# kepengxu/RealCamNet

Hardware: AMD Instinct MI355X
Metric: megapixels/sec RAW->sRGB at 4K (higher is better)
Workload: dtype bf16; 1 GPU; cfg3: 3840x2160 Bayer mosaic -> unshuffle+pad16 -> LiteISPNet_GFM_LSC_GMA -> sRGB 3840x2160, 8 frames/GPU, bf16 storage / fp32 accumulate; frames_per_gpu=8, global_frames=8, parallelism=frame-shard x1, collective=none

## Files before the change

### realcamnet_amd/csrc/conv.hip

```cpp
#include <mutex>
#include <vector>

#include "conv32_kernel.hpp"

namespace rc {

struct ConvPlan {
    int ck = 0, nt = 0, unit = 0, upt = 0, nu = 0, steps = 0;
    int n_chunks = 0, n_ct = 0, cout_packed = 0;
    int m32 = 0;
};

static int g_persist_on = 1;
extern int g_dw3_seg16;
extern int g_dec_lds;
extern int g_wmsa_mfma;
extern int g_pw_grid_cap;
static int g_pss = 0;
static int g_poison = 0;
static int g_thin = 2;
static int g_auto = 1;
static int g_sums_compact = 1;
static int g_conv32 = 0;

static bool make_plan(int cin, int cout, int ksize, int dtype, int out_mode, ConvPlan* p, int cout_tile = 0) {
    if (cin < 1 || cout < 1 || (ksize != 1 && ksize != 3 && ksize != 2 && ksize != 5)) return false;
    if (dtype != RC_F32 && dtype != RC_BF16 && dtype != RC_F16) return false;
    const bool h16 = dtype != RC_F32;
    if (ksize == 5 && (cout > 16 || out_mode == RC_OUT_PIXEL_SHUFFLE2 || (h16 ? (cin % 48 != 0 && cin % 32 != 0) : cin % 16 != 0))) return false;
    if (out_mode == RC_OUT_PIXEL_SHUFFLE2_NCHW && cout % 4 != 0) return false;
    if (ksize == 2 && (dtype != RC_BF16 || cin % 16 != 0 || out_mode != RC_OUT_NHWC || (cin % 48 == 0 && cin % 64 != 0))) return false;
    p->unit = dtype == RC_F32 ? 4 : 8;
    if (ksize == 5) p->ck = h16 ? (cin % 48 == 0 ? 48 : 32) : 16;
    else if (h16) {
        if (cin <= 8) p->ck = 8;
        else if (ksize == 1 && cin % 80 == 0 && cin % 64 != 0) p->ck = 80;
        else if (ksize >= 2 && cin % 64 == 0 && cin > 64) p->ck = 32;
        else if (cin % 64 == 0) p->ck = 64;
        else if (cin % 48 == 0) p->ck = 48;
        else if (ksize == 3 && cin == 32) p->ck = 32;
        else if (ksize == 3 && cin % 32 == 0 && cin > 64) p->ck = 32;
        else p->ck = 16;
    } else {
        p->ck = cin <= 4 ? 4 : 16;
    }
    if (out_mode == RC_OUT_PIXEL_SHUFFLE2) {
        if (cout % 4 != 0) return false;
        const int cps = cout / 4;
        if (cps % 64 == 0 && !(cps % 48 == 0 && h16 && cin == 48)) p->nt = 4;
        else if (cps % 48 == 0) p->nt = 3;
        else if (cps % 64 == 0) p->nt = 4;
        else if (cps % 16 == 0) p->nt = 1;
        else return false;
// ... 181 lines not shown
                    for (int dx = 0; dx < 3; ++dx) {
                        const int a = i + dy - 1, b = j + dx - 1;
                        const int fy = a < 0 ? -1 : a >> 1, ii = a & 1, fx = b < 0 ? -1 : b >> 1, jj = b & 1;
                        for (int cc = 0; cc < c; ++cc) {
                            const int m = 4 * cc + 2 * ii + jj;
                            const double v2 = w2[(((size_t)oo * c + cc) * 3 + dy) * 3 + dx];
                            if (b1) bacc[row] += v2 * (double)b1[m];
                            for (int k = 0; k < c; ++k)
                                for (int ey = 0; ey < 3; ++ey)
                                    for (int ex = 0; ex < 3; ++ex)
                                        acc[(((size_t)row * c + k) * 5 + (fy + ey + 1)) * 5 + (fx + ex + 1)] += v2 * (double)w1[(((size_t)m * c + k) * 3 + ey) * 3 + ex];
                        }
                    }
            }
    for (size_t n = 0; n < acc.size(); ++n) wc[n] = (float)acc[n];
    for (size_t n = 0; n < bacc.size(); ++n) bc[n] = (float)bacc[n];
    return RC_OK;
}

int rc_conv_sum_tiles(int height, int width) { return 4 * ceil_div(height, kTH) * ceil_div(width, kTW); }

int rc_debug_set(const char* key, int value) {
    RC_REQUIRE(key != nullptr, "rc_debug_set: null key");
    if (std::string(key) == "persist") { g_persist_on = value < 0 ? 0 : (value > 3 ? 3 : value); return RC_OK; }
    if (std::string(key) == "conv_flags") { g_dbg_flags = value; return RC_OK; }
    if (std::string(key) == "pair_impl") { g_pair_impl = value < 0 || value > 2 ? 0 : value; return RC_OK; }
    if (std::string(key) == "dec_lds") { g_dec_lds = value != 0; return RC_OK; }
    if (std::string(key) == "dw3_seg16") { g_dw3_seg16 = value != 0; return RC_OK; }
    if (std::string(key) == "wmsa_mfma") { g_wmsa_mfma = value != 0; return RC_OK; }
    if (std::string(key) == "pss") { g_pss = value != 0; return RC_OK; }
    if (std::string(key) == "sums_compact") { g_sums_compact = value != 0; return RC_OK; }
    if (std::string(key) == "persist_auto") { g_auto = value < 0 ? 0 : (value > 2 ? 2 : value); return RC_OK; }
    if (std::string(key) == "thin") { g_thin = value < 0 ? 0 : (value > 2 ? 2 : value); return RC_OK; }
    if (std::string(key) == "lds_poison") { g_poison = value != 0; return RC_OK; }
    if (std::string(key) == "conv32") { g_conv32 = value < 0 ? 0 : (value > 4 ? 4 : value); return RC_OK; }
    if (std::string(key) == "wino_nnt") { wino_set_nnt(value); return RC_OK; }
    if (std::string(key) == "pw_grid_cap") { g_pw_grid_cap = value <= 0 || value > (1 << 22) ? (1 << 22) : value; return RC_OK; }
    return fail(RC_ERR_INVALID, std::string("rc_debug_set: unknown key ") + key);
}

int rc_debug_get(const char* key) {
    if (key == nullptr) return -1;
    if (std::string(key) == "persist") return g_persist_on;
    if (std::string(key) == "conv32") return g_conv32;
    if (std::string(key) == "conv_flags") return g_dbg_flags;
    if (std::string(key) == "pss") return g_pss;
    if (std::string(key) == "sums_compact") return g_sums_compact;
    if (std::string(key) == "persist_auto") return g_auto;
    if (std::string(key) == "thin") return g_thin;
    if (std::string(key) == "lds_poison") return g_poison;
    if (std::string(key) == "wino_nnt") return wino_get_nnt();
    if (std::string(key) == "pw_grid_cap") return g_pw_grid_cap;
    return -1;
}

int rc_debug_set_ptr(const char* key, void* p) {
    RC_REQUIRE(key != nullptr, "rc_debug_set_ptr: null key");
    if (std::string(key) == "conv_phase_timing") { g_dbg_ptr = static_cast<long long*>(p); return RC_OK; }
    return fail(RC_ERR_INVALID, std::string("rc_debug_set_ptr: unknown key ") + key);
}

int rc_prof_enable(int on) {
    std::lock_guard<std::mutex> lk(g_prof_mu);
    for (auto& r : g_prof) { (void)hipEventDestroy(r.e0); (void)hipEventDestroy(r.e1); }
    g_prof.clear();
    g_prof_on = on != 0;
    return RC_OK;
}

int rc_prof_collect(int64_t* n_launches, double* total_ms, double* total_flops) {
    std::lock_guard<std::mutex> lk(g_prof_mu);
    double ms = 0.0, fl = 0.0;
    for (auto& r : g_prof) {
        RC_HIP_CHECK(hipEventSynchronize(r.e1));
        float t = 0.f;
        RC_HIP_CHECK(hipEventElapsedTime(&t, r.e0, r.e1));
        ms += t; fl += r.flops;
    }
    if (n_launches) *n_launches = (int64_t)g_prof.size();
    if (total_ms) *total_ms = ms;
    if (total_flops) *total_flops = fl;
    return RC_OK;
// ... 98 lines not shown
    a.cin_vec_ok = (d->cin % p.unit == 0) && aligned16(d->in0) && aligned16(d->in1) && aligned16(d->in_store) &&
                   (d->in_gate == nullptr || reinterpret_cast<uintptr_t>(d->in_gate) % 4 == 0);
    a.cin_chunk_ok = d->cin % p.ck == 0;
    a.fold2 = fold ? 1 : 0; a.src_H = d->src_h; a.src_W = d->src_w; a.cfold = d->cin / 4;
    a.in0 = d->in0; a.in1 = d->in1; a.in_gate = d->in_gate; a.in_store = d->in_store;
    a.wpacked = d->wpacked; a.bias = d->bias;
    a.film_scale = d->film_scale; a.film_shift = d->film_shift;
    a.act = d->act; a.act_slope = d->act_slope;
    a.mul_plus1 = d->mul_plus1; a.residual = d->residual; a.out_scale = d->out_scale;
    a.out = d->out; a.out_mode = d->out_mode; a.out_dtype = d->out_dtype; a.out_h = d->out_h; a.out_w = d->out_w;
    a.chan_sums = d->chan_sums; a.cout_packed = p.cout_packed;
    a.sum_slots = d->chan_sums_slots > 0 ? d->chan_sums_slots : 4 * ceil_div(d->height, kTH) * ceil_div(d->width, kTW);
    a.sums_compact = 0; a.query = nullptr; a.sums_compact_ok = g_sums_compact;
    {
        int key = (d->act == RC_ACT_RELU ? 1 : 0) | (d->act == RC_ACT_LEAKY ? 2 : 0) | (d->film_scale ? 4 : 0) |
                  (d->mul_plus1 ? 8 : 0) | (d->residual ? 16 : 0) | (d->chan_sums ? 32 : 0) | (d->out_scale ? 64 : 0);
        bool fast = full_tiles && d->out_mode != RC_OUT_NCHW && d->out_mode != RC_OUT_PIXEL_SHUFFLE2_NCHW && d->act != RC_ACT_GELU && d->act != RC_ACT_RELU_POST;
        if (d->act == RC_ACT_LEAKY) fast = fast && d->act_slope >= 0.f && d->act_slope <= 1.f;
        if (d->film_scale)
            fast = fast && d->cout % 4 == 0 && reinterpret_cast<uintptr_t>(d->film_scale) % 16 == 0 && reinterpret_cast<uintptr_t>(d->film_shift) % 16 == 0;
        if (d->out_scale) fast = fast && d->cout % 4 == 0 && reinterpret_cast<uintptr_t>(d->out_scale) % 16 == 0;
        switch (key) { case 0: case 1: case 2: case 16: case 32: case 8: case 6: case 33: case 34: case 80: break; default: fast = false; }
        a.ep_key = fast ? key : -1;
        a.pss = g_pss && d->out_mode == RC_OUT_PIXEL_SHUFFLE2 && !p.m32 && p.n_chunks == 1 && p.n_ct == 4 && d->cout == 4 * 16 * p.nt &&
                d->dtype == RC_BF16 && d->in_gate == nullptr && fast && (key == 0 || key == 1 || key == 2);
    }
    {
        const int num_cus = device_cu_count();
        a.num_cus = num_cus;
        a.persist_ok = g_persist_on;
        a.auto_impl = g_auto;
        a.thin = g_thin;
        a.dbg = g_dbg_ptr;
        a.dbg_flags = g_dbg_flags;
        a.td = make_tile_decode(a.tiles_x, a.tiles_y, kBandRows);
        a.td_wsm = make_tile_decode(a.tiles_x, (a.H + kWsmTH - 1) / kWsmTH, kBandRows);
        a.div_n_ct = make_magic(a.n_ct);
    }
    es_out = es;
    return RC_OK;
}

int rc_conv2d(const rc_conv_desc* d, void* stream_) {
    RC_REQUIRE(d != nullptr, "rc_conv2d: null desc");
    RC_REQUIRE(d->algo == 0 || d->algo == 1, "rc_conv2d: algo must be 0 (implicit GEMM) or 1 (Winograd F(2x2,3x3))");
    if (d->algo == 1) {
        if (g_poison) { if (int e = rc_debug_poison_lds(0x7FC07FC0u, stream_)) return e; }
        return wino_conv(d, as_stream(stream_));
    }
    ConvPlan p;
    ConvArgs a;
    size_t es = 0;
    if (int e = conv_build_args(d, p, a, es)) return e;
    hipStream_t stream = as_stream(stream_);
    if (g_poison) { if (int e = rc_debug_poison_lds(0x7FC07FC0u, stream_)) return e; }
    void* tok = nullptr;
    const double taps = d->ksize == 2 ? 9.0 / 4.0 : (double)d->ksize * d->ksize;
    const double px = (double)d->batch * d->height * d->width;
    const double osz = (d->out_mode == RC_OUT_NCHW || d->out_mode == RC_OUT_PIXEL_SHUFFLE2_NCHW) ? (d->out_dtype == RC_F32 ? 4.0 : 2.0) : (double)es;
    const double bytes = px * d->cin * es * (1.0 + (d->in1 ? 1.0 : 0.0) + (d->in_store ? 1.0 : 0.0)) + px * d->cout * osz +
                         px * d->cout * es * ((d->residual ? 1.0 : 0.0) + (d->mul_plus1 ? 1.0 : 0.0));
    conv_prof_begin(2.0 * px * (double)d->cin * d->cout * taps, stream, &tok, bytes, d->cin, d->cout, d->ksize);
    const int rcode = p.m32 ? (p.ck == 16 ? conv32_ck16(0, a, stream) : p.ck == 32 ? conv32_ck32(g_conv32 == 3 ? 1 : 0, a, stream) : conv32_ck48(0, a, stream))
                            : dispatch_conv(d->dtype, d->ksize, p.ck, p.nt, a, stream);
    conv_prof_end(tok, stream);
    return rcode;
}
// ... 17 lines not shown
```

### realcamnet_amd/csrc/conv_kernel.hpp

```cpp
#pragma once
#include "common.hpp"

namespace rc {

struct MagicDiv { unsigned m, sh; };
inline MagicDiv make_magic(int d) {
    if (d <= 1) return MagicDiv{0u, 0u};
    int L = 0;
    while ((2 << L) <= d) ++L;
    const unsigned long long m = ((1ull << (31 + L)) + (unsigned long long)d - 1) / (unsigned long long)d;
    return MagicDiv{(unsigned)m, (unsigned)(L - 1)};
}
__device__ __forceinline__ int magic_div(int n, const MagicDiv& d) {
    return d.m ? (int)(__umulhi((unsigned)n, d.m) >> d.sh) : n;
}
struct TileDecode { MagicDiv sp_total, band, last_rows; };
inline TileDecode make_tile_decode(int tiles_x, int tiles_y, int band_rows) {
    return TileDecode{make_magic(tiles_x * tiles_y), make_magic(band_rows * tiles_x), make_magic(tiles_y % band_rows ? tiles_y % band_rows : 1)};
}

struct ConvArgs {
    int batch, H, W, cin, cout;
    int n_chunks, n_ct, tiles_x, tiles_y;
    int cin_vec_ok;
    int cin_chunk_ok;
    const void* in0; const void* in1; const float* in_gate; void* in_store;
    const void* wpacked; const float* bias;
    const float* film_scale; const float* film_shift;
    int act; float act_slope;
    const void* mul_plus1; const void* residual;
    const float* out_scale;
    void* out; int out_mode; int out_dtype; int out_h, out_w;
    float* chan_sums; int cout_packed;
    int sum_slots;
    int sums_compact_ok;
    int sums_compact;
    int* query;
    int num_cus; int persist_ok;
    int ep_key;
    TileDecode td, td_wsm;
    MagicDiv div_n_ct;
    int w_resident;
    int pss;
    int auto_impl;
    int thin;
    int fold2, src_H, src_W, cfold;
    long long* dbg;
    int dbg_flags;
};

constexpr int kTH = 8, kTW = 32, kThreads = 256;

constexpr int pix_stride_bytes(int ck_bytes) {
    int s = (ck_bytes + 15) / 16 * 16;
    while (s % 64 != 32) s += 16;
    return s;
}

__host__ __device__ constexpr int unit_map_steps(int upt, int taps) {
    return upt == 6 ? taps + (taps + 1) / 2 : (taps * upt + 3) / 4;
}
__host__ __device__ constexpr bool unit_map(int upt, int taps, int s, int q, int& tap, int& cu) {
    if (upt == 6) {
        if (s < taps) { tap = s; cu = q; return true; }
        tap = 2 * (s - taps) + (q >> 1); cu = 4 + (q & 1);
        return tap < taps;
    }
    const int u = 4 * s + q;
    tap = u / upt; cu = u % upt;
    return u < taps * upt;
}

template <typename T, int CK_, int NT_, int KS_, int TH_ = kTH>
struct ConvCfg {
    using elem = T;
    static constexpr int CK = CK_, NT = NT_, KS = KS_, TH = TH_;
    static constexpr int UNIT = 16 / (int)sizeof(T);
    static_assert(CK % UNIT == 0, "CK must be a whole number of 16-byte units");
    static constexpr int UPT = CK / UNIT;
    static constexpr int TAPS = KS * KS;
    static constexpr int STEPS = unit_map_steps(UPT, TAPS);
    static constexpr int HALO = KS / 2;
// ... 80 lines not shown
            __builtin_amdgcn_raw_buffer_store_b64(u32x2_t{w[4 * NQ], w[4 * NQ + 1]}, r, voff + 16 * NQ, 0, 0);
    }
}

template <typename TT, int NV>
__device__ __forceinline__ void buf_load_row(__amdgpu_buffer_rsrc_t r, int voff, float* v) {
    if constexpr (sizeof(TT) == 4) {
#pragma unroll
        for (int i = 0; i < NV; i += 4) {
            const u32x4_t t = __builtin_amdgcn_raw_buffer_load_b128(r, voff + 4 * i, 0, 0);
            v[i] = __uint_as_float(t.x); v[i + 1] = __uint_as_float(t.y); v[i + 2] = __uint_as_float(t.z); v[i + 3] = __uint_as_float(t.w);
        }
    } else {
#pragma unroll
        for (int i = 0; i < NV; i += 4) {
            const u32x2_t p = __builtin_amdgcn_raw_buffer_load_b64(r, voff + 2 * i, 0, 0);
            v[i] = lo16<TT>(p.x); v[i + 1] = hi16<TT>(p.x);
            v[i + 2] = lo16<TT>(p.y); v[i + 3] = hi16<TT>(p.y);
        }
    }
}

constexpr int kBandRows = 8;
__device__ __forceinline__ void band_decode(int idx, int tiles_x, int tiles_y, const TileDecode& td, int& ty, int& tx) {
    const int band = magic_div(idx, td.band);
    const int rem = idx - band * (kBandRows * tiles_x);
    const int rows_left = tiles_y - band * kBandRows;
    const bool whole = rows_left >= kBandRows;
    const int col = whole ? rem >> 3 : magic_div(rem, td.last_rows);
    ty = band * kBandRows + (rem - col * (whole ? kBandRows : rows_left));
    tx = col;
}

template <class Cfg>
struct ConvDev {
    using T = typename Cfg::elem;
    using TS = typename std::conditional<sizeof(T) == 4, bf16_t, T>::type;
    static constexpr int CK = Cfg::CK, NT = Cfg::NT, KS = Cfg::KS, UNIT = Cfg::UNIT, UPT = Cfg::UPT, TAPS = Cfg::TAPS;
    static constexpr int STEPS = Cfg::STEPS, HALO = Cfg::HALO, THH = Cfg::THH, TWH = Cfg::TWH;
    static constexpr int SPIX = Cfg::SPIX, NV = 4 * NT, ES = (int)sizeof(T);
    static constexpr int VPP = UPT;
    static constexpr int NPIX = THH * TWH;
    static constexpr int PPP = kThreads / VPP;
    static constexpr int ACTIVE = PPP * VPP;
    static constexpr int NI = (NPIX + PPP - 1) / PPP;
    static constexpr bool TABLE = (UPT % 4 != 0) && (UPT != 6);

    __device__ static constexpr int tap_off(int tap) { return ((tap / KS) * TWH + (tap % KS)) * SPIX; }

    struct LaneOff {
        int a;
        int b;
        int c;
        int tab[TABLE ? STEPS : 1];
    };
    __device__ static __forceinline__ void lane_offsets(int q, LaneOff& lo) {
        lo.a = q * 16;
        lo.b = (q >> 1) * SPIX + (4 + (q & 1)) * 16;
        lo.c = (q >> 1) * (TWH - (KS - 1)) * SPIX + (4 + (q & 1)) * 16;
        if constexpr (TABLE) {
#pragma unroll
            for (int s = 0; s < STEPS; ++s) {
                int tap = 0, cu = 0;
                if (!unit_map(UPT, TAPS, s, q, tap, cu)) { tap = TAPS - 1; cu = UPT - 1; }
                lo.tab[s] = tap_off(tap) + cu * 16;
            }
        } else {
            lo.tab[0] = 0;
        }
    }
    __device__ static __forceinline__ int step_off(int s, const LaneOff& lo) {
        if constexpr (TABLE) {
            return lo.tab[s];
        } else if constexpr (UPT == 6) {
            if (s < TAPS) return lo.a + tap_off(s);
            const int t0 = 2 * (s - TAPS);
            const bool wrap = (t0 + 1 < TAPS) && ((t0 + 1) % KS == 0);
            return (wrap ? lo.c : lo.b) + tap_off(t0);
        } else {
            const int u = 4 * s;
            return lo.a + tap_off(u / UPT) + (u % UPT) * 16;
        }
    }
    __device__ static constexpr bool step_has_pad(int s) {
        int tap = 0, cu = 0;
        return !unit_map(UPT, TAPS, s, 3, tap, cu);
    }
    __device__ static __forceinline__ bool lane_is_pad(int s, int q) {
        if constexpr (UPT == 6) return q >= 2;
        else return 4 * s + q >= TAPS * UPT;
    }

    struct TileSrc {
        __amdgpu_buffer_rsrc_t r0, r1, rst;
        int gy0, gx0;
        int soff;
        bool interior;
// ... 73 lines not shown
        }
    }
    template <bool GATED>
    __device__ static __forceinline__ void load_tile_interior(const ConvArgs& a, const TileSrc& t, const TileOffs& to, int chunk,
                                                              uint4 (&r0)[NI], uint4 (&r1)[GATED ? NI : 1]) {
        const int soff = t.soff + chunk_soff(a, chunk);
#pragma unroll
        for (int k = 0; k < NI; ++k) {
            r0[k] = buf_load16(t.r0, to.o[k], soff);
            if constexpr (GATED) r1[k] = buf_load16(t.r1, to.o[k], soff);
        }
    }
    template <bool GATED>
    __device__ static __forceinline__ void load_tile_border(const ConvArgs& a, const TileSrc& t, int chunk, int tid,
                                                            uint4 (&r0)[NI], uint4 (&r1)[GATED ? NI : 1]) {
        const int v = tid % VPP, p0 = tid / VPP;
        const bool live = tid < ACTIVE;
#pragma unroll
        for (int k = 0; k < NI; ++k) {
            bool center;
            const int off = vec_off(a, t, chunk, p0 + k * PPP, v, live, center);
            r0[k] = buf_load16(t.r0, off, 0);
            if constexpr (GATED) r1[k] = buf_load16(t.r1, off, 0);
        }
    }

    template <bool GATED>
    __device__ static __forceinline__ void commit_tile(const ConvArgs& a, const TileSrc& t, const TileOffs& to, int chunk, int tid,
                                                       const uint4 (&r0)[NI], const uint4 (&r1)[GATED ? NI : 1],
                                                       const float (&gv)[GATED ? UNIT : 1], char* s_in) {
        const int v = tid % VPP, p0 = tid / VPP;
        const bool live = tid < ACTIVE;
        char* dst = s_in + p0 * SPIX + v * 16;
#pragma unroll
        for (int k = 0; k < NI; ++k) {
            const int pix = p0 + k * PPP;
            uint4 raw = r0[k];
            if constexpr (GATED) {
                float f0[UNIT], f1[UNIT];
                Vec16<T>::unpack(r0[k], f0);
                Vec16<T>::unpack(r1[k], f1);
#pragma unroll
                for (int e = 0; e < UNIT; ++e) f0[e] = f0[e] * gv[e] + f1[e];
                raw = Vec16<T>::pack(f0);
                if (t.interior) {
                    buf_store16(t.rst, to.ctr[k], t.soff + chunk * CK * ES, raw);
                } else {
                    bool center;
                    const int off = vec_off(a, t, chunk, pix, v, live, center);
                    buf_store16(t.rst, center ? off : kOOB, 0, raw);
                }
            }
            if (live && pix < NPIX) *reinterpret_cast<uint4*>(dst + k * PPP * SPIX) = raw;
        }
    }

    __device__ static __forceinline__ void stage_tile_scalar(const ConvArgs& a, int b, int y0, int x0, int chunk, int tid,
                                                             char* s_in, T* in_store) {
        const T* in0 = static_cast<const T*>(a.in0);
        const T* in1 = static_cast<const T*>(a.in1);
        const size_t img_base = (size_t)b * a.H * a.W;
        if constexpr (ES == 2 && UNIT == 8 && VPP == 1) {
            if (a.cin == 4 && a.in_gate == nullptr && (reinterpret_cast<uintptr_t>(in0) & 7) == 0) {
                for (int i = tid; i < NPIX; i += kThreads) {
                    const int py = i / TWH, px = i - py * TWH;
                    const int gy = y0 + py - HALO, gx = x0 + px - HALO;
// ... 21 lines not shown
                    if (c0 + e < a.cin) {
                        val = to_f32(in0[off + e]);
                        if (a.in_gate != nullptr)
                            val = val * a.in_gate[(size_t)b * a.cin + c0 + e] + to_f32(in1[off + e]);
                    }
                    f0[e] = val;
                }
                raw = Vec16<T>::pack(f0);
                if (a.in_gate != nullptr && in_store != nullptr && center) {
#pragma unroll
                    for (int e = 0; e < UNIT; ++e)
                        if (c0 + e < a.cin) in_store[off + e] = from_f32<T>(f0[e]);
                }
            }
            *reinterpret_cast<uint4*>(s_in + pix * SPIX + v * 16) = raw;
        }
    }

    __device__ static __forceinline__ void dma_weights(const char* src, char* dst, int nkb, int wave, int lane_w) {
        for (int kb = wave; kb < nkb; kb += kThreads / 64)
            __builtin_amdgcn_global_load_lds((const __attribute__((address_space(1))) void*)(src + kb * 1024 + lane_w),
                                             (__attribute__((address_space(3))) void*)(dst + kb * 1024), 16, 0, 0);
    }

    static constexpr int FR = NT + 4;
    static constexpr int FM = 4 * NT;
    template <int I>
    __device__ static __forceinline__ void load_frag_item(int s, int w0, const char* s_in, const char* s_w, int lane_x,
                                                          int lane_w, const LaneOff& lo, uint4 (&wf)[NT], uint4 (&xf)[4]) {
        if constexpr (I < NT) {
            wf[I] = *reinterpret_cast<const uint4*>(s_w + ((s - w0) * NT + I) * 1024 + lane_w);
        } else {
            constexpr int pt = I - NT;
            xf[pt] = *reinterpret_cast<const uint4*>(s_in + lane_x + step_off(s, lo) + ((pt >> 1) * TWH + (pt & 1) * 16) * SPIX);
        }
    }
    __device__ static __forceinline__ void zero_pad_frags(int s, int q, uint4 (&xf)[4]) {
        if (step_has_pad(s)) {
            if (lane_is_pad(s, q)) {
#pragma unroll
                for (int pt = 0; pt < 4; ++pt) xf[pt] = make_uint4(0u, 0u, 0u, 0u);
            }
        }
    }
    __device__ static __forceinline__ void load_frags(int s, int w0, const char* s_in, const char* s_w, int lane_x,
                                                      int lane_w, int q, const LaneOff& lo, uint4 (&wf)[NT], uint4 (&xf)[4]) {
#pragma unroll
        for (int nt = 0; nt < NT; ++nt)
            wf[nt] = *reinterpret_cast<const uint4*>(s_w + ((s - w0) * NT + nt) * 1024 + lane_w);
        const char* xp = s_in + lane_x + step_off(s, lo);
#pragma unroll
        for (int pt = 0; pt < 4; ++pt)
            xf[pt] = *reinterpret_cast<const uint4*>(xp + ((pt >> 1) * TWH + (pt & 1) * 16) * SPIX);
        zero_pad_frags(s, q, xf);
    }
    __device__ static __forceinline__ void mma_frags(const uint4 (&wf)[NT], const uint4 (&xf)[4], f32x4 (&acc)[4][NT]) {
#pragma unroll
        for (int pt = 0; pt < 4; ++pt)
#pragma unroll
            for (int nt = 0; nt < NT; ++nt) Mma<T>::run(wf[nt], xf[pt], acc[pt][nt]);
    }
    static constexpr int SLOTS = FM * (ES == 4 ? 4 : 1);
    __device__ static __forceinline__ void mma_slot(int m, const uint4 (&wf)[NT], const uint4 (&xf)[4], f32x4 (&acc)[4][NT]) {
        if constexpr (ES == 4) {
            const int e = m / FM, j = m % FM, pt = j / NT, nt = j % NT;
            const unsigned w = e == 0 ? wf[nt].x : e == 1 ? wf[nt].y : e == 2 ? wf[nt].z : wf[nt].w;
            const unsigned x = e == 0 ? xf[pt].x : e == 1 ? xf[pt].y : e == 2 ? xf[pt].z : xf[pt].w;
            acc[pt][nt] = __builtin_amdgcn_mfma_f32_16x16x4f32(__uint_as_float(w), __uint_as_float(x), acc[pt][nt], 0, 0, 0);
        } else {
            Mma<T>::run(wf[m % NT], xf[m / NT], acc[m / NT][m % NT]);
        }
    }
    template <int I, bool NEXT>
    __device__ static __forceinline__ void step_interleaved(int s, int w0, const char* s_in, const char* s_w, int lane_x, int lane_w,
                                                            const LaneOff& lo, const uint4 (&wf)[NT], const uint4 (&xf)[4],
                                                            uint4 (&wfn)[NT], uint4 (&xfn)[4], f32x4 (&acc)[4][NT]) {
        if constexpr (I < FR) {
            if constexpr (NEXT) load_frag_item<I>(s + 1, w0, s_in, s_w, lane_x, lane_w, lo, wfn, xfn);
            if constexpr (ES == 2) __builtin_amdgcn_sched_barrier(0);
#pragma unroll
            for (int m = (I * SLOTS) / FR; m < ((I + 1) * SLOTS) / FR; ++m) mma_slot(m, wf, xf, acc);
            if constexpr (ES == 2) __builtin_amdgcn_sched_barrier(0);
            step_interleaved<I + 1, NEXT>(s, w0, s_in, s_w, lane_x, lane_w, lo, wf, xf, wfn, xfn, acc);
        }
    }
    template <int S0, int COUNT, int W0, bool DBUF = true>
    __device__ static __forceinline__ void mma_steps(const char* s_in, const char* s_w, int lane_x, int lane_w, int q,
                                                     const LaneOff& lo, f32x4 (&acc)[4][NT]) {
        constexpr int END = (S0 + COUNT) < STEPS ? (S0 + COUNT) : STEPS;
        if constexpr (S0 < END && !DBUF) {
#pragma unroll
            for (int s = S0; s < END; ++s) {
                uint4 wf[NT], xf[4];
                load_frags(s, W0, s_in, s_w, lane_x, lane_w, q, lo, wf, xf);
                mma_frags(wf, xf, acc);
            }
        } else if constexpr (S0 < END && ES == 4) {
            uint4 wfa[NT], xfa[4], wfb[NT], xfb[4];
            load_frags(S0, W0, s_in, s_w, lane_x, lane_w, q, lo, wfa, xfa);
#pragma unroll
            for (int s = S0; s < END; s += 2) {
                if (s + 1 < END) load_frags(s + 1, W0, s_in, s_w, lane_x, lane_w, q, lo, wfb, xfb);
                mma_frags(wfa, xfa, acc);
                if (s + 2 < END) load_frags(s + 2, W0, s_in, s_w, lane_x, lane_w, q, lo, wfa, xfa);
                if (s + 1 < END) mma_frags(wfb, xfb, acc);
            }
        } else if constexpr (S0 < END) {
            uint4 wfa[NT], xfa[4], wfb[NT], xfb[4];
            load_frags(S0, W0, s_in, s_w, lane_x, lane_w, q, lo, wfa, xfa);
#pragma unroll
            for (int s = S0; s < END; s += 2) {
                if (s + 1 < END) step_interleaved<0, true>(s, W0, s_in, s_w, lane_x, lane_w, lo, wfa, xfa, wfb, xfb, acc);
                else step_interleaved<0, false>(s, W0, s_in, s_w, lane_x, lane_w, lo, wfa, xfa, wfb, xfb, acc);
                if (s + 1 < END) {
                    zero_pad_frags(s + 1, q, xfb);
                    if (s + 2 < END) step_interleaved<0, true>(s + 1, W0, s_in, s_w, lane_x, lane_w, lo, wfb, xfb, wfa, xfa, acc);
                    else step_interleaved<0, false>(s + 1, W0, s_in, s_w, lane_x, lane_w, lo, wfb, xfb, wfa, xfa, acc);
                    if (s + 2 < END) zero_pad_frags(s + 2, q, xfa);
                }
            }
        }
    }
// ... 966 lines not shown
                        const char* s_in = s_in0 + (one_chunk ? (k & 1) : (g & 1)) * Cfg::IN_BYTES;
                        if constexpr (ph == 3) { if (!(a.dbg_flags & 2)) D::template mma_steps<0, SA, 0, true>(s_in, s_w, lane_x, lane_w, q, lo, acc); }
                        else if constexpr (ph == 2) D::template mma_steps<1, 1, 0, false>(s_in, s_w, lane_x, lane_w, q, lo, acc);
                        __syncthreads();
                        if constexpr ((ph & 1) != 0) { if (!(a.dbg_flags & 2)) D::template mma_steps<SA, STEPS - SA, 0, true>(s_in, s_w, lane_x, lane_w, q, lo, acc); }
                        else D::template mma_steps<3, 1, 0, false>(s_in, s_w, lane_x, lane_w, q, lo, acc);
                        if (c + 1 < n_chunks) __syncthreads();
                    }
                };
                if constexpr (FOLD_SKIP) {
                    const int cpp = D::folded(a) ? n_chunks >> 2 : 0;
                    run_chunks(std::integral_constant<int, 0>{}, 0, cpp);
                    run_chunks(std::integral_constant<int, 1>{}, cpp, 2 * cpp);
                    run_chunks(std::integral_constant<int, 2>{}, 2 * cpp, 3 * cpp);
                    run_chunks(std::integral_constant<int, 3>{}, 3 * cpp, n_chunks);
                } else {
                    run_chunks(std::integral_constant<int, 3>{}, 0, n_chunks);
                }
                if (ty8 < a.tiles_y)
                    D8::template epilogue<FAST>(a, b, ty8 * kTH, tx * kTW, ty8 * a.tiles_x + tx, ct, tid & 255, acc);
                __syncthreads();
            }
        }
    }
}

template <class Cfg8>
struct WstCfg : WsmCfg<Cfg8> {
    using B = WsmCfg<Cfg8>;
    static constexpr int SPIX = B::CK * (int)sizeof(typename B::elem);
    static constexpr int N_PIECES = B::THH * B::TWH * B::UPT;
    static constexpr int N_DMA = (N_PIECES + 63) / 64;
    static constexpr int IN_BYTES = N_DMA * 1024;
};
template <class Cfg>
constexpr int wst_form() {
    if (!(sizeof(typename Cfg::elem) == 2 && (Cfg::KS == 2 || Cfg::KS == 3) && (Cfg::UPT == 2 || Cfg::UPT == 4) && Cfg::STEPS >= 2)) return 0;
    const int w = (int)Cfg::CHUNK_W_BYTES, in = WstCfg<Cfg>::IN_BYTES, fixed = 2 * w + kPersistMaxCout * 4;
    if (w <= 20 * 1024 && fixed + 3 * in <= 160 * 1024) return 3;
    if (w <= 36 * 1024 && fixed + 2 * in <= 160 * 1024) return 2;
    return 0;
}
template <class Cfg>
constexpr int wst_lds_bytes() { return 2 * (int)Cfg::CHUNK_W_BYTES + kPersistMaxCout * 4 + (wst_form<Cfg>() == 3 ? 3 : 2) * WstCfg<Cfg>::IN_BYTES; }
template <class Cfg>
constexpr bool wst_eligible() { return wst_form<Cfg>() != 0; }
constexpr int waitcnt_vm(int n) { return (n & 15) | ((n >> 4) << 14) | 0x0F70; }

template <class Cfg8, bool FAST>
__global__ __launch_bounds__(kWsmThreads) void conv_mfma_wst_kernel(const ConvArgs a) {
#if defined(__HIP_DEVICE_COMPILE__)
    using Cfg = WstCfg<Cfg8>;
    using D = ConvDev<Cfg>;
    using D8 = ConvDev<Cfg8>;
    constexpr int NT = Cfg::NT, STEPS = Cfg::STEPS, NV = 4 * NT, WALL = (int)Cfg::CHUNK_W_BYTES, UPT = Cfg::UPT, TWH = Cfg::TWH, ES = 2;
    constexpr int N_DMA = Cfg::N_DMA, NDW = (N_DMA + 3) / 4;
    constexpr int NBUF = wst_form<Cfg8>() == 3 ? 3 : 2;
    constexpr bool FOLD_SKIP = Cfg::KS == 2 && UPT == 4 && STEPS == 4;

    extern __shared__ __attribute__((aligned(16))) char smem[];
    char* s_w = smem;
    float* s_bias = reinterpret_cast<float*>(smem + 2 * WALL);
    char* s_in0 = smem + 2 * WALL + kPersistMaxCout * 4;

    const int tid = threadIdx.x, lane = tid & 63;
    const int wave12 = __builtin_amdgcn_readfirstlane(tid >> 6);
// ... 34 lines not shown
            int k_unit = 0, cti = 0, chunk = 0, gi = 0, ct = 0;
            int b = 0, ty = 0, tx = 0, ct0 = 0;
            auto fetch = [&]() {
                if (gi < my_stages) {
                    if (chunk == 0) {
                        if (cti == 0) decode(pos + k_unit * stride, b, ty, tx, ct0);
                        ct = ct0 + cti;
                        ts = D::tile_src(a, b, ty * kWsmTH, tx * kTW);
                    }
                    const int goff = (ct * n_chunks + chunk) * WALL;
                    for (int kb = w4; kb < WALL / 1024; kb += 4)
                        __builtin_amdgcn_global_load_lds((const __attribute__((address_space(1))) void*)(static_cast<const char*>(a.wpacked) + goff + kb * 1024 + lane * 16),
                                                         (__attribute__((address_space(3))) void*)(s_w + (gi & 1) * WALL + kb * 1024), 16, 0, 0);
                    if (!one_chunk || cti == 0) {
                        D::template load_tile<false>(a, ts, to, b, chunk, rtid, r0, r1, gv);
                        D::template commit_tile<false>(a, ts, to, chunk, rtid, r0, r1, gv, s_in0 + (one_chunk ? (k_unit & 1) : (gi & 1)) * Cfg::IN_BYTES);
                    }
                }
                ++gi;
                if (++chunk == n_chunks) { chunk = 0; if (++cti == cts_per_unit) { cti = 0; ++k_unit; } }
            };
            fetch();
            __syncthreads();
            for (int g = 0; g < my_stages; ++g) {
                fetch();
                __syncthreads();
            }
        }
    } else if (loader) {
        const int w4 = wave12 - 8;
        int lc[NDW];
#pragma unroll
        for (int r = 0; r < NDW; ++r) {
            const int P = (w4 + 4 * r) * 64 + lane, pix = P / UPT, v = P - pix * UPT, py = pix / TWH, px = pix - py * TWH;
            const int o = D::folded(a) ? ((2 * py * a.src_W + 2 * px) * a.cfold + v * Cfg::UNIT) * ES : ((py * a.W + px) * a.cin + v * Cfg::UNIT) * ES;
            lc[r] = P < Cfg::N_PIECES ? o : kOOB;
        }
        typename D::TileSrc ts;
        int k_unit = 0, cti = 0, chunk = 0, gi = 0, gb3 = 0, kb3 = 0;
        int b = 0, ty = 0, tx = 0, ct0 = 0;
        const int n_mine = (N_DMA - w4 + 3) / 4;
        auto issue = [&]() -> int {
            const bool tile = gi < my_stages && (!one_chunk || cti == 0);
            char* dst = s_in0 + (one_chunk ? kb3 : gb3) * Cfg::IN_BYTES;
            int in_flight = 0;
            if (tile && chunk == 0) {
                decode(pos + k_unit * stride, b, ty, tx, ct0);
                ts = D::tile_src(a, b, ty * kWsmTH, tx * kTW);
            }
            if (tile && ts.interior) {
                const int soff = ts.soff + D::chunk_soff(a, chunk);
#pragma unroll
                for (int r = 0; r < NDW; ++r) {
                    const int inst = w4 + 4 * r;
                    if (inst < N_DMA)
                        __builtin_amdgcn_raw_ptr_buffer_load_lds(ts.r0, (__attribute__((address_space(3))) void*)(dst + inst * 1024), 16, lc[r], soff, 0, 0);
                }
                in_flight = n_mine;
            } else if (tile) {
                int ln = lane;
                asm volatile("" : "+v"(ln));
#pragma unroll
                for (int r = 0; r < NDW; ++r) {
                    const int inst = w4 + 4 * r, P = inst * 64 + ln, pix = P / UPT, v = P - pix * UPT;
                    if (inst < N_DMA) {
                        bool center;
                        const int off = P < Cfg::N_PIECES ? D::vec_off(a, ts, chunk, pix, v, true, center) : kOOB;
                        __builtin_amdgcn_raw_ptr_buffer_load_lds(ts.r0, (__attribute__((address_space(3))) void*)(dst + inst * 1024), 16, off, 0, 0, 0);
                    }
                }
            }
            ++gi; gb3 = gb3 == 2 ? 0 : gb3 + 1;
            if (++chunk == n_chunks) { chunk = 0; if (++cti == cts_per_unit) { cti = 0; ++k_unit; kb3 = kb3 == 2 ? 0 : kb3 + 1; } }
            return in_flight;
        };
        int wi = 0, wk = 0, wcti = 0, wchunk = 0, wct0 = 0;
        auto issue_w = [&]() {
            if (wi < my_stages) {
                if (wchunk == 0 && wcti == 0) { int b_, ty_, tx_; decode(pos + wk * stride, b_, ty_, tx_, wct0); }
                const int goff = ((wct0 + wcti) * n_chunks + wchunk) * WALL;
                int ph = 3;
                if constexpr (FOLD_SKIP) ph = D::folded(a) ? D::fold_phase(a, wchunk * Cfg::CK) : 3;
                for (int kb = w4; kb < WALL / 1024; kb += 4) {
                    if constexpr (FOLD_SKIP) {
                        const int st = kb / NT;
                        if (!(st == 3 || ph == 3 || (ph == 1 && st == 2) || (ph == 2 && st == 1))) continue;
                    }
                    __builtin_amdgcn_global_load_lds((const __attribute__((address_space(1))) void*)(static_cast<const char*>(a.wpacked) + goff + kb * 1024 + lane * 16),
                                                     (__attribute__((address_space(3))) void*)(s_w + (wi & 1) * WALL + kb * 1024), 16, 0, 0);
                }
            }
            ++wi;
            if (++wchunk == n_chunks) { wchunk = 0; if (++wcti == cts_per_unit) { wcti = 0; ++wk; } }
        };
        issue_w();
        issue();
        issue();
        __syncthreads();
        for (int g = 0; g < my_stages; ++g) {
            issue_w();
            const int nfl = issue();
            if (nfl == NDW) __builtin_amdgcn_s_waitcnt(waitcnt_vm(NDW));
            else if (NDW > 1 && nfl == NDW - 1) __builtin_amdgcn_s_waitcnt(waitcnt_vm(NDW > 1 ? NDW - 1 : 0));
            else __builtin_amdgcn_s_waitcnt(waitcnt_vm(0));
            __builtin_amdgcn_s_barrier();
        }
        __builtin_amdgcn_s_waitcnt(waitcnt_vm(0));
    } else {
        const int wave = wave12;
        typename D::LaneOff lo;
        D::lane_offsets(q, lo);
        const int lane_x = ((2 * wave) * D::TWH + n) * D::SPIX;
        const int lane_w = lane * 16;
        __syncthreads();
        int g = 0, gb3 = 0, kb3 = 0;
        for (int k = 0; k < my_units; ++k) {
            int b, ty, tx, ct0;
            decode(pos + k * stride, b, ty, tx, ct0);
            const int ty8 = 2 * ty + (wave >> 2);
            for (int ct = ct0; ct < ct0 + cts_per_unit; ++ct) {
                f32x4 acc[4][NT];
#pragma unroll
                for (int nt = 0; nt < NT; ++nt) {
                    const float4 t4 = *reinterpret_cast<const float4*>(s_bias + ct * Cfg::COUT_TILE + q * NV + nt * 4);
#pragma unroll
                    for (int pt = 0; pt < 4; ++pt) acc[pt][nt] = f32x4{t4.x, t4.y, t4.z, t4.w};
                }
                auto run_chunks = [&](auto PH, int c0, int c1) {
                    constexpr int ph = decltype(PH)::value;
                    for (int c = c0; c < c1; ++c, ++g) {
                        const char* s_in = s_in0 + (one_chunk ? kb3 : gb3) * Cfg::IN_BYTES;
                        const char* s_wg = s_w + (g & 1) * WALL;
                        if constexpr (ph == 3) D::template mma_steps<0, STEPS, 0, true>(s_in, s_wg, lane_x, lane_w, q, lo, acc);
                        else if constexpr (ph == 1) D::template mma_steps<2, 2, 0, true>(s_in, s_wg, lane_x, lane_w, q, lo, acc);
                        else {
                            if constexpr (ph == 2) D::template mma_steps<1, 1, 0, false>(s_in, s_wg, lane_x, lane_w, q, lo, acc);
                            D::template mma_steps<3, 1, 0, false>(s_in, s_wg, lane_x, lane_w, q, lo, acc);
                        }
                        gb3 = gb3 == NBUF - 1 ? 0 : gb3 + 1;
                        if (c + 1 < n_chunks) __syncthreads();
                    }
                };
                if constexpr (FOLD_SKIP) {
                    const int cpp = D::folded(a) ? n_chunks >> 2 : 0;
// ... 699 lines not shown
```

Baseline: 1344 MP/s.

## Swizzle LDS input tile layout for WST conv to avoid bank conflicts

Adds an XOR swizzle to the LDS placement of input pieces for the UPT==4 WST conv configuration. The DMA piece mapping, the cooperative tile writes and the fragment reads are all remapped consistently, with per-stage precomputed lane offsets. The aim is to remove LDS bank conflicts on the 16-byte fragment reads that feed MFMA. In exchange it adds index arithmetic and eight extra registers per lane, and it is switchable through a debug flag.

```diff
diff --git a/realcamnet_amd/csrc/conv.hip b/realcamnet_amd/csrc/conv.hip
--- a/realcamnet_amd/csrc/conv.hip
+++ b/realcamnet_amd/csrc/conv.hip
@@ -19,6 +19,7 @@
 static int g_pss = 0;
 static int g_poison = 0;
 static int g_thin = 2;
+static int g_wst_swizzle = 1;
 static int g_auto = 1;
 static int g_sums_compact = 1;
 static int g_conv32 = 0;
@@ -266,6 +267,7 @@
     if (std::string(key) == "sums_compact") { g_sums_compact = value != 0; return RC_OK; }
     if (std::string(key) == "persist_auto") { g_auto = value < 0 ? 0 : (value > 2 ? 2 : value); return RC_OK; }
     if (std::string(key) == "thin") { g_thin = value < 0 ? 0 : (value > 2 ? 2 : value); return RC_OK; }
+    if (std::string(key) == "wst_swizzle") { g_wst_swizzle = value != 0; return RC_OK; }
     if (std::string(key) == "lds_poison") { g_poison = value != 0; return RC_OK; }
     if (std::string(key) == "conv32") { g_conv32 = value < 0 ? 0 : (value > 4 ? 4 : value); return RC_OK; }
     if (std::string(key) == "wino_nnt") { wino_set_nnt(value); return RC_OK; }
@@ -282,6 +284,7 @@
     if (std::string(key) == "sums_compact") return g_sums_compact;
     if (std::string(key) == "persist_auto") return g_auto;
     if (std::string(key) == "thin") return g_thin;
+    if (std::string(key) == "wst_swizzle") return g_wst_swizzle;
     if (std::string(key) == "lds_poison") return g_poison;
     if (std::string(key) == "wino_nnt") return wino_get_nnt();
     if (std::string(key) == "pw_grid_cap") return g_pw_grid_cap;
@@ -446,7 +449,7 @@
         a.auto_impl = g_auto;
         a.thin = g_thin;
         a.dbg = g_dbg_ptr;
-        a.dbg_flags = g_dbg_flags;
+        a.dbg_flags = (g_dbg_flags & ~kWstLinear) | (g_wst_swizzle ? 0 : kWstLinear);
         a.td = make_tile_decode(a.tiles_x, a.tiles_y, kBandRows);
         a.td_wsm = make_tile_decode(a.tiles_x, (a.H + kWsmTH - 1) / kWsmTH, kBandRows);
         a.div_n_ct = make_magic(a.n_ct);
diff --git a/realcamnet_amd/csrc/conv_kernel.hpp b/realcamnet_amd/csrc/conv_kernel.hpp
--- a/realcamnet_amd/csrc/conv_kernel.hpp
+++ b/realcamnet_amd/csrc/conv_kernel.hpp
@@ -1,5 +1,6 @@
 #pragma once
 #include "common.hpp"
+#include "lds_layout.hpp"
 
 namespace rc {
 
@@ -48,6 +49,8 @@
     long long* dbg;
     int dbg_flags;
 };
+constexpr int kWstLinear = 1 << 16;
+__host__ __device__ inline bool wst_swz_on(const ConvArgs& a) { return (a.dbg_flags & kWstLinear) == 0; }
 
 constexpr int kTH = 8, kTW = 32, kThreads = 256;
 
@@ -194,9 +197,15 @@
     tx = col;
 }
 
+template <class C, class = void> struct cfg_lds_dense : std::false_type {};
+template <class C> struct cfg_lds_dense<C, std::void_t<decltype(C::LDS_DENSE)>> : std::integral_constant<bool, C::LDS_DENSE> {};
+template <class C, class = void> struct cfg_lds_swz : std::false_type {};
+template <class C> struct cfg_lds_swz<C, std::void_t<decltype(C::LDS_SWZ)>> : std::integral_constant<bool, C::LDS_SWZ> {};
+
 template <class Cfg>
 struct ConvDev {
     using T = typename Cfg::elem;
+    static constexpr bool LDS_DENSE = cfg_lds_dense<Cfg>::value, LDS_SWZ = cfg_lds_swz<Cfg>::value;
     using TS = typename std::conditional<sizeof(T) == 4, bf16_t, T>::type;
     static constexpr int CK = Cfg::CK, NT = Cfg::NT, KS = Cfg::KS, UNIT = Cfg::UNIT, UPT = Cfg::UPT, TAPS = Cfg::TAPS;
     static constexpr int STEPS = Cfg::STEPS, HALO = Cfg::HALO, THH = Cfg::THH, TWH = Cfg::TWH;
@@ -210,12 +219,36 @@
 
     __device__ static constexpr int tap_off(int tap) { return ((tap / KS) * TWH + (tap % KS)) * SPIX; }
 
-    struct LaneOff {
+    struct SwzOff {
+        const char* base;
+        int lin;
+        int on;
+        int x[8];
+    };
+    struct NoSwzOff {};
+    struct LaneOff : std::conditional<LDS_SWZ, SwzOff, NoSwzOff>::type {
         int a;
         int b;
         int c;
         int tab[TABLE ? STEPS : 1];
     };
+    __device__ static __forceinline__ void swz_lane(const char* s_in0, int wave, int n, int q, int on, LaneOff& lo) {
+        if constexpr (LDS_SWZ) { lo.base = s_in0; lo.lin = ldsmap::wst_lane_lin(UPT, TWH, wave, n, q); lo.on = on; }
+    }
+    __device__ static __forceinline__ LaneOff swz_stage(const char* s_in, const LaneOff& lo) {
+        LaneOff ls = lo;
+        {
+            static_assert(UPT == 4 && !TABLE, "swizzled reads: a step is the four units of one tap");
+            const int rel = lo.lin + (int)(s_in - lo.base);
+#pragma unroll
+            for (int r = 0; r < 8; ++r) ls.x[r] = ldsmap::wst_place(UPT, rel + r * SPIX, lo.on != 0);
+        }
+        return ls;
+    }
+    __device__ static __forceinline__ uint4 read_xfrag(int s, int pt, const char* s_in, int lane_x, const LaneOff& lo) {
+        const int c = ldsmap::wst_frag_pix(KS, TWH, s, pt);
+        return *reinterpret_cast<const uint4*>(lo.base + lo.x[ldsmap::wst_read_reg(c)] + ldsmap::wst_read_imm(c));
+    }
     __device__ static __forceinline__ void lane_offsets(int q, LaneOff& lo) {
         lo.a = q * 16;
         lo.b = (q >> 1) * SPIX + (4 + (q & 1)) * 16;
@@ -224,7 +257,10 @@
 #pragma unroll
             for (int s = 0; s < STEPS; ++s) {
                 int tap = 0, cu = 0;
-                if (!unit_map(UPT, TAPS, s, q, tap, cu)) { tap = TAPS - 1; cu = UPT - 1; }
+                if (!unit_map(UPT, TAPS, s, q, tap, cu)) {
+                    tap = TAPS - 1; cu = UPT - 1;
+                    if constexpr (LDS_DENSE) cu = ldsmap::wst_pad_unit(UPT, q);
+                }
                 lo.tab[s] = tap_off(tap) + cu * 16;
             }
         } else {
@@ -364,6 +400,10 @@
         const int v = tid % VPP, p0 = tid / VPP;
         const bool live = tid < ACTIVE;
         char* dst = s_in + p0 * SPIX + v * 16;
+        if constexpr (LDS_SWZ) {
+            static_assert((PPP * SPIX) % ldsmap::kWstPeriod == 0, "swizzled tile: passes must keep the slot");
+            dst = s_in + ldsmap::wst_write_off(UPT, p0, v, wst_swz_on(a));
+        }
 #pragma unroll
         for (int k = 0; k < NI; ++k) {
             const int pix = p0 + k * PPP;
@@ -451,7 +491,8 @@
             wf[I] = *reinterpret_cast<const uint4*>(s_w + ((s - w0) * NT + I) * 1024 + lane_w);
         } else {
             constexpr int pt = I - NT;
-            xf[pt] = *reinterpret_cast<const uint4*>(s_in + lane_x + step_off(s, lo) + ((pt >> 1) * TWH + (pt & 1) * 16) * SPIX);
+            if constexpr (LDS_SWZ) xf[pt] = read_xfrag(s, pt, s_in, lane_x, lo);
+            else xf[pt] = *reinterpret_cast<const uint4*>(s_in + lane_x + step_off(s, lo) + ((pt >> 1) * TWH + (pt & 1) * 16) * SPIX);
         }
     }
     __device__ static __forceinline__ void zero_pad_frags(int s, int q, uint4 (&xf)[4]) {
@@ -467,10 +508,15 @@
 #pragma unroll
         for (int nt = 0; nt < NT; ++nt)
             wf[nt] = *reinterpret_cast<const uint4*>(s_w + ((s - w0) * NT + nt) * 1024 + lane_w);
-        const char* xp = s_in + lane_x + step_off(s, lo);
-#pragma unroll
-        for (int pt = 0; pt < 4; ++pt)
-            xf[pt] = *reinterpret_cast<const uint4*>(xp + ((pt >> 1) * TWH + (pt & 1) * 16) * SPIX);
+        if constexpr (LDS_SWZ) {
+#pragma unroll
+            for (int pt = 0; pt < 4; ++pt) xf[pt] = read_xfrag(s, pt, s_in, lane_x, lo);
+        } else {
+            const char* xp = s_in + lane_x + step_off(s, lo);
+#pragma unroll
+            for (int pt = 0; pt < 4; ++pt)
+                xf[pt] = *reinterpret_cast<const uint4*>(xp + ((pt >> 1) * TWH + (pt & 1) * 16) * SPIX);
+        }
         zero_pad_frags(s, q, xf);
     }
     __device__ static __forceinline__ void mma_frags(const uint4 (&wf)[NT], const uint4 (&xf)[4], f32x4 (&acc)[4][NT]) {
@@ -505,8 +551,11 @@
     }
     template <int S0, int COUNT, int W0, bool DBUF = true>
     __device__ static __forceinline__ void mma_steps(const char* s_in, const char* s_w, int lane_x, int lane_w, int q,
-                                                     const LaneOff& lo, f32x4 (&acc)[4][NT]) {
+                                                     const LaneOff& lo_, f32x4 (&acc)[4][NT]) {
         constexpr int END = (S0 + COUNT) < STEPS ? (S0 + COUNT) : STEPS;
+        typename std::conditional<LDS_SWZ, LaneOff, char>::type ls{};
+        if constexpr (LDS_SWZ) ls = swz_stage(s_in, lo_);
+        const LaneOff& lo = [&]() -> const LaneOff& { if constexpr (LDS_SWZ) return ls; else return lo_; }();
         if constexpr (S0 < END && !DBUF) {
 #pragma unroll
             for (int s = S0; s < END; ++s) {
@@ -1539,6 +1588,9 @@
     static constexpr int N_PIECES = B::THH * B::TWH * B::UPT;
     static constexpr int N_DMA = (N_PIECES + 63) / 64;
     static constexpr int IN_BYTES = N_DMA * 1024;
+    static constexpr bool LDS_DENSE = true;
+    static constexpr bool LDS_SWZ = ldsmap::wst_swizzled(B::UPT);
+    static_assert(!LDS_SWZ || N_PIECES % 4 == 0, "the swizzle moves a piece inside its pixel");
 };
 template <class Cfg>
 constexpr int wst_form() {
@@ -1639,7 +1691,8 @@
         int lc[NDW];
 #pragma unroll
         for (int r = 0; r < NDW; ++r) {
-            const int P = (w4 + 4 * r) * 64 + lane, pix = P / UPT, v = P - pix * UPT, py = pix / TWH, px = pix - py * TWH;
+            const int P = ldsmap::wst_dma_piece(UPT, (w4 + 4 * r) * 64 + lane, wst_swz_on(a));
+            const int pix = P / UPT, v = P - pix * UPT, py = pix / TWH, px = pix - py * TWH;
             const int o = D::folded(a) ? ((2 * py * a.src_W + 2 * px) * a.cfold + v * Cfg::UNIT) * ES : ((py * a.W + px) * a.cin + v * Cfg::UNIT) * ES;
             lc[r] = P < Cfg::N_PIECES ? o : kOOB;
         }
@@ -1669,7 +1722,7 @@
                 asm volatile("" : "+v"(ln));
 #pragma unroll
                 for (int r = 0; r < NDW; ++r) {
-                    const int inst = w4 + 4 * r, P = inst * 64 + ln, pix = P / UPT, v = P - pix * UPT;
+                    const int inst = w4 + 4 * r, P = ldsmap::wst_dma_piece(UPT, inst * 64 + ln, wst_swz_on(a)), pix = P / UPT, v = P - pix * UPT;
                     if (inst < N_DMA) {
                         bool center;
                         const int off = P < Cfg::N_PIECES ? D::vec_off(a, ts, chunk, pix, v, true, center) : kOOB;
@@ -1717,6 +1770,7 @@
         const int wave = wave12;
         typename D::LaneOff lo;
         D::lane_offsets(q, lo);
+        D::swz_lane(s_in0, wave, n, q, wst_swz_on(a), lo);
         const int lane_x = ((2 * wave) * D::TWH + n) * D::SPIX;
         const int lane_w = lane * 16;
         __syncthreads();
diff --git a/realcamnet_amd/csrc/lds_layout.hpp b/realcamnet_amd/csrc/lds_layout.hpp
--- /dev/null
+++ b/realcamnet_amd/csrc/lds_layout.hpp
@@ -0,0 +1,33 @@
+#pragma once
+
+#if defined(__HIPCC__)
+#define RC_LDS_FN __host__ __device__ constexpr
+#else
+#define RC_LDS_FN constexpr
+#endif
+
+namespace rc {
+namespace ldsmap {
+
+RC_LDS_FN int wst_lin(int upt, int pix, int v) { return (pix * upt + v) * 16; }
+
+RC_LDS_FN bool wst_swizzled(int upt) { return upt == 4; }
+
+RC_LDS_FN int wst_place(int upt, int lin, bool on) { return (on && wst_swizzled(upt)) ? (lin ^ ((lin >> 3) & 32)) : lin; }
+
+constexpr int kWstPeriod = 512;
+
+RC_LDS_FN int wst_write_off(int upt, int pix, int v, bool on) { return wst_place(upt, wst_lin(upt, pix, v), on); }
+RC_LDS_FN int wst_dma_piece(int upt, int slot, bool on) { return wst_place(upt, slot * 16, on) >> 4; }
+
+RC_LDS_FN int wst_lane_lin(int upt, int twh, int wave, int n, int v) { return wst_lin(upt, 2 * wave * twh + n, v); }
+RC_LDS_FN int wst_frag_pix(int ks, int twh, int tap, int pt) { return (tap / ks + (pt >> 1)) * twh + tap % ks + (pt & 1) * 16; }
+RC_LDS_FN int wst_pad_unit(int upt, int q) { return q % upt; }
+RC_LDS_FN int wst_read_reg(int c) { return c & 7; }
+RC_LDS_FN int wst_read_imm(int c) { return (c >> 3) * kWstPeriod; }
+RC_LDS_FN int wst_read_off(int upt, int lane_lin, int c, bool on) {
+    return wst_swizzled(upt) ? wst_place(upt, lane_lin + 16 * upt * wst_read_reg(c), on) + wst_read_imm(c) : lane_lin + 16 * upt * c;
+}
+
+}
+}
```

Result: no change. 1338 MP/s (-0.4%).
